# hailanyi/CPD

Measured on AMD Instinct MI355X. Metric: frames/sec voxelize->sparse3D->BEV->NMS, 160k-pt Waymo cloud, higher is better.
Workload: dtype f32 (split-fp16 x2 on the fp16 MFMA pipe: 3 products, fp32 accumulate)

## Files before the change

cpd_amd/_lib.py:

```python
import ctypes
import os

import torch

_HERE = os.path.dirname(os.path.abspath(__file__))
LIB_PATH = os.environ.get("CPD_HIP_LIB", os.path.join(_HERE, "csrc", "libcpd_hip.so"))

CPD_ERRORS = {-1: "CPD_ERR_ARG", -2: "CPD_ERR_WORKSPACE", -3: "CPD_ERR_LAUNCH", -4: "CPD_ERR_UNSUPPORTED"}


class CpdHipError(RuntimeError):
    pass


_lib = None

_VP, _I, _F, _SZ = ctypes.c_void_p, ctypes.c_int, ctypes.c_float, ctypes.c_size_t
_D = ctypes.c_double
_I3 = ctypes.POINTER(ctypes.c_int32)
_FP = ctypes.POINTER(ctypes.c_float)

SIGNATURES = {
    "cpd_launch_log_enable": (None, [_I]),
    "cpd_launch_log_note": (None, [ctypes.c_char_p]),
# ... 4 lines not shown
    "cpd_voxelize_workspace_bytes": (_SZ, [_I, _I, _I, _FP, _FP]),
    "cpd_voxelize_batch_workspace_bytes": (_SZ, [_I, _I, _I, _I, _FP, _FP]),
    "cpd_voxelize_batch": (_I, [_VP, _I3, _I, _I, _FP, _FP, _I, _I, _VP, _VP, _VP, _VP, _VP, _VP, _SZ, _VP]),
    "cpd_voxelize_batch_index": (_I, [_VP, _I3, _I, _I, _FP, _FP, _I, _I, _VP, _VP, _VP, _VP, _VP, _VP, _SZ, _VP, _SZ, _I, _VP]),
    "cpd_voxelize_batch_canonical": (_I, [_VP, _I3, _I, _I, _FP, _FP, _I, _I, _VP, _VP, _VP, _VP, _VP, _VP, _SZ, _VP, _SZ, _I, _VP]),
    "cpd_voxelize_batch_frames": (_I, [_VP, _I3, _I, _I, _FP, _FP, _I, _I, _VP, _VP, _VP, _VP, _VP, _VP, _SZ, _VP, _SZ, _I, _I, _VP]),
    "cpd_voxelize": (_I, [_VP, _I, _I, _FP, _FP, _I, _I, _I, _I, _VP, _VP, _VP, _VP, _VP, _VP, _SZ, _VP]),
    "cpd_index_bytes": (_SZ, [_I, _I3, _I]),
    "cpd_index_build": (_I, [_VP, _I, _I, _I3, _VP, _SZ, _VP]),
    "cpd_order_rows_by_taps_workspace_bytes": (_SZ, [_I]),
    "cpd_order_rows_by_taps": (_I, [_VP, _I, _I, _I3, _I3, _VP, _I, _VP, _VP, _VP, _VP, _SZ, _VP]),
    "cpd_index_set_order": (_I, [_VP, _VP, _VP]),
    "cpd_order_rows_bricks_workspace_bytes": (_SZ, [_I]),
    "cpd_order_rows_bricks": (_I, [_VP, _I, _I, _I3, _VP, _I, _I, _I, _VP, _VP, _VP, _VP, _SZ, _VP]),
    "cpd_rulebook_chunk_ordered": (_I, [_VP, _VP, _I, _I, _I3, _I3, _I3, _I3, _VP, _I, _VP, _VP, _VP]),
    "cpd_rulebook_plan_bytes": (_SZ, [_I, _I, _I]),
    "cpd_rulebook_plan": (_I, [_VP, _I, _I, _I, _VP, _VP, _VP, _VP]),
    "cpd_gather_conv_planned_supported": (_I, [_I, _I, _I, _I, _I, _I, _I]),
    "cpd_gather_conv_planned": (_I, [_VP, _I, _I, _I, _VP, _VP, _VP, _VP, _VP, _I, _I, _I, _I, _VP, _VP, _VP, _I, _I, _VP, _I, _I, _VP, _VP]),
    "cpd_rulebook_subm": (_I, [_VP, _I, _I, _I3, _I3, _VP, _VP, _VP, _VP]),
    "cpd_conv_out_shape": (_I, [_I3, _I3, _I3, _I3, _I3]),
    "cpd_conv_outset": (_I, [_VP, _I, _I, _I3, _I3, _I3, _I3, _VP, _SZ, _VP, _VP]),
    "cpd_index_emit": (_I, [_VP, _I, _I3, _VP, _I, _VP]),
    "cpd_rulebook_conv": (_I, [_VP, _I, _I, _I3, _I3, _I3, _I3, _VP, _VP, _VP, _VP]),
    "cpd_packed_weight_floats": (_SZ, [_I, _I, _I]),
    "cpd_pack_weight": (_I, [_VP, _I, _I, _I, _VP, _VP]),
    "cpd_gather_conv": (_I, [_VP, _I, _I, _I, _VP, _VP, _VP, _I, _I, _I, _VP, _VP, _VP, _I, _I, _VP, _I, _VP, _I, _I, _VP]),
    "cpd_gather_conv_scaled": (_I, [_VP, _I, _I, _I, _VP, _VP, _VP, _I, _I, _I, _VP, _VP, _VP, _I, _I, _VP, _I, _VP, _I, _I, _VP, _VP]),
    "cpd_gather_conv_tile": (_I, [_I, _I, _I, _I, _I] + [ctypes.POINTER(_I)] * 4),
    "cpd_gather_conv_label": (ctypes.c_char_p, [_I, _I, _I, _I, _I, _I, _I]),
# ... 217 lines not shown
```

cpd_amd/csrc/site_index.hip:

```cpp
#include "common.h"

#include "site_index_layout.h"

namespace {

__global__ void __launch_bounds__(256) index_mark_kernel(const int32_t *__restrict__ idx, int n, Grid g, uint64_t *bitmap) {
    int i = blockIdx.x * blockDim.x + threadIdx.x;
    if (i >= n) return;
    int4 q = reinterpret_cast<const int4 *>(idx)[i];
    if ((unsigned)q.x >= (unsigned)g.b || (unsigned)q.y >= (unsigned)g.d || (unsigned)q.z >= (unsigned)g.h ||
        (unsigned)q.w >= (unsigned)g.w)
        return;
    long long k = g.key(q.x, q.y, q.z, q.w);
    atomicOr((unsigned long long *)&bitmap[k >> 6], 1ull << (k & 63));
}

__global__ void __launch_bounds__(256) index_perm_kernel(const int32_t *__restrict__ idx, int n, Grid g,
                                                         const uint64_t *__restrict__ bitmap,
                                                         const uint32_t *__restrict__ base, int32_t *perm) {
    int i = blockIdx.x * blockDim.x + threadIdx.x;
    if (i >= n) return;
    int4 q = reinterpret_cast<const int4 *>(idx)[i];
    if ((unsigned)q.x >= (unsigned)g.b || (unsigned)q.y >= (unsigned)g.d || (unsigned)q.z >= (unsigned)g.h ||
        (unsigned)q.w >= (unsigned)g.w)
// ... 6 lines not shown
    const uint64_t *bitmap;
    __device__ uint32_t operator()(long long w) const { return (uint32_t)__popcll(bitmap[w]); }
};
struct StoreBaseFn {
    uint32_t *base;
    __device__ void operator()(long long w, uint32_t, uint32_t prefix) const { base[w] = prefix; }
};
struct EmitFn {
    const uint64_t *bitmap;
    const uint32_t *base;
    int32_t *out;
    int n_cap;
    Grid g;
    __device__ void operator()(long long wi, uint32_t, uint32_t) const {
        uint64_t w = bitmap[wi];
        uint32_t r = base[wi];
        while (w) {
            int bpos = __ffsll((unsigned long long)w) - 1;
            w &= w - 1;
            long long k = wi * 64 + bpos;
            if ((int)r < n_cap) {
                int x = (int)(k % g.w);
                long long t = k / g.w;
                int y = (int)(t % g.h);
                t /= g.h;
                int z = (int)(t % g.d);
                int bi = (int)(t / g.d);
                reinterpret_cast<int4 *>(out)[r] = make_int4(bi, z, y, x);
            }
            ++r;
        }
    }
};

#pragma clang diagnostic push
#pragma clang diagnostic ignored "-Wpass-failed"
template <bool K3>
__global__ void __launch_bounds__(256)
rulebook_kernel(const int32_t *__restrict__ out_idx, int n_out, Grid gin, int kd_, int kh_, int kw_, int sd, int sh, int sw,
                int pd, int ph, int pw, const uint64_t *__restrict__ bitmap, const uint32_t *__restrict__ base,
                const int32_t *__restrict__ perm_in, const int32_t *__restrict__ flags, int32_t *__restrict__ nbr,
                uint32_t *__restrict__ tapmask, uint32_t *__restrict__ row_pattern) {
    int j = blockIdx.x * blockDim.x + threadIdx.x;
    const int kd = K3 ? 3 : kd_, kh = K3 ? 3 : kh_, kw = K3 ? 3 : kw_;
// ... 11 lines not shown
    for (int tz = 0; tz < kd; ++tz) {
        int z = q.y * sd - pd + tz;
#pragma unroll
        for (int ty = 0; ty < kh; ++ty) {
            int y = q.z * sh - ph + ty;
            const bool row_ok = (unsigned)z < (unsigned)gin.d && (unsigned)y < (unsigned)gin.h && (unsigned)q.x < (unsigned)gin.b &&
                                xlo <= xhi;
            long long rowkey = 0;
            uint64_t wa = 0, wb = 0;
            uint32_t ba = 0, bb = 0;
            long long wia = 0;
            if (row_ok) {
                rowkey = gin.key(q.x, z, y, 0);
                wia = (rowkey + xlo) >> 6;
                const long long wib = (rowkey + xhi) >> 6;
                wa = bitmap[wia]; ba = base[wia];
                wb = wa; bb = ba;
                if (wib != wia) { wb = bitmap[wib]; bb = base[wib]; }
            }
#pragma unroll
            for (int tx = 0; tx < kw; ++tx, ++t) {
                int x = x0 + tx;
                int32_t r = -1;
                if (row_ok && (unsigned)x < (unsigned)gin.w) {
                    const long long k = rowkey + x;
                    const bool first = (k >> 6) == wia;
                    const uint64_t w = first ? wa : wb;
                    const uint64_t bit = 1ull << (k & 63);
                    if (w & bit) {
                        r = (int32_t)((first ? ba : bb) + __popcll(w & (bit - 1ull)));
                        if (perm) r = perm[r];
                    }
                }
                if (live && nbr) nbr[(size_t)t * n_out + j] = r;
                if (r >= 0 && t < 32) pattern |= 1u << t;
                const unsigned long long hit = __ballot(live && r >= 0);
                if (lane < 4 && t < 32 && ((hit >> (16 * lane)) & 0xffffull)) my_mask |= 1u << t;
            }
        }
    }
    if (tapmask && lane < 4) {
        const int sub = ((blockIdx.x * blockDim.x + (threadIdx.x & ~63)) >> 4) + lane;
        if (sub < (n_out + 15) / 16) tapmask[sub] = my_mask;
    }
    if (row_pattern && live) row_pattern[j] = pattern;
}

#pragma clang diagnostic pop

#define CPD_RBC_CHUNK 4096
__global__ void __launch_bounds__(1024)
rulebook_chunk_kernel(const int32_t *__restrict__ out_canon, const int32_t *__restrict__ out_o2n, int n_out, Grid gin, int sd, int sh, int sw,
                      int pd, int ph, int pw, const uint64_t *__restrict__ bitmap, const uint32_t *__restrict__ base,
                      const int32_t *__restrict__ perm_in, const int32_t *__restrict__ flags, int32_t *__restrict__ nbr,
                      uint32_t *__restrict__ tapmask) {
    __shared__ int32_t stage[3][CPD_RBC_CHUNK];
    constexpr int RPT = CPD_RBC_CHUNK / 1024;
    const int tid = threadIdx.x;
    const int c0 = blockIdx.x * CPD_RBC_CHUNK;
    const int32_t *perm = index_order(flags, perm_in);
    int4 q[RPT];
    int dst[RPT];
#pragma unroll
    for (int k = 0; k < RPT; ++k) {
        const int j = c0 + k * 1024 + tid;
        dst[k] = -1;
        q[k] = make_int4(0, 0, 0, 0);
        if (j < n_out) {
            q[k] = reinterpret_cast<const int4 *>(out_canon)[j];
            dst[k] = (out_o2n ? out_o2n[j] : j) - c0;
        }
    }
    uint32_t pattern[RPT];
#pragma unroll
    for (int k = 0; k < RPT; ++k) pattern[k] = 0;
    for (int tzy = 0; tzy < 9; ++tzy) {
        const int tz = tzy / 3, ty = tzy - 3 * tz;
#pragma unroll
        for (int k = 0; k < RPT; ++k) {
            if (dst[k] < 0) continue;
            const int z = q[k].y * sd - pd + tz, y = q[k].z * sh - ph + ty;
            const int x0 = q[k].w * sw - pw;
            int32_t r3[3] = {-1, -1, -1};
            if ((unsigned)z < (unsigned)gin.d && (unsigned)y < (unsigned)gin.h && (unsigned)q[k].x < (unsigned)gin.b) {
                const long long rowkey = gin.key(q[k].x, z, y, 0);
                const int xlo = x0 < 0 ? 0 : x0, xhi = x0 + 2 < gin.w ? x0 + 2 : gin.w - 1;
                if (xlo <= xhi) {
                    const long long wia = (rowkey + xlo) >> 6, wib = (rowkey + xhi) >> 6;
                    const uint64_t wa = bitmap[wia];
                    const uint32_t ba = base[wia];
                    uint64_t wb = wa;
                    uint32_t bb = ba;
                    if (wib != wia) { wb = bitmap[wib]; bb = base[wib]; }
#pragma unroll
                    for (int tx = 0; tx < 3; ++tx) {
                        const int x = x0 + tx;
                        if ((unsigned)x >= (unsigned)gin.w) continue;
                        const long long kk = rowkey + x;
                        const bool first = (kk >> 6) == wia;
                        const uint64_t w = first ? wa : wb;
                        const uint64_t bit = 1ull << (kk & 63);
                        if (w & bit) {
                            int32_t r = (int32_t)((first ? ba : bb) + __popcll(w & (bit - 1ull)));
                            if (perm) r = perm[r];
                            r3[tx] = r;
                        }
                    }
                }
            }
#pragma unroll
            for (int tx = 0; tx < 3; ++tx) stage[tx][dst[k]] = r3[tx];
        }
        __syncthreads();
#pragma unroll
        for (int k = 0; k < RPT; ++k) {
            const int i = k * 1024 + tid, row = c0 + i;
            if (row < n_out) {
#pragma unroll
                for (int tx = 0; tx < 3; ++tx) {
                    const int32_t v = stage[tx][i];
                    nbr[(size_t)(3 * tzy + tx) * n_out + row] = v;
                    if (v >= 0) pattern[k] |= 1u << (3 * tzy + tx);
                }
            }
        }
        __syncthreads();
    }
    if (tapmask) {
#pragma unroll
        for (int k = 0; k < RPT; ++k) {
            uint32_t m = pattern[k];
#pragma unroll
            for (int o = 8; o > 0; o >>= 1) m |= (uint32_t)__shfl_xor((int)m, o, 16);
            const int row = c0 + k * 1024 + tid;
            if ((tid & 15) == 0 && row < n_out) tapmask[row >> 4] = m;
        }
    }
}

__device__ __forceinline__ void outset_flush(uint64_t *bitmap, long long word, uint64_t mask, bool valid) {
    const int lane = threadIdx.x & 63;
    long long key = valid ? word : -1 - lane;
#pragma unroll
    for (int d = 1; d < 64; d <<= 1) {
        const long long k2 = __shfl_up(key, d, 64);
        const uint64_t m2 = __shfl_up(mask, d, 64);
        if (lane >= d && k2 == key) mask |= m2;
    }
    const long long kn = __shfl_down(key, 1, 64);
    const bool tail = lane == 63 || kn != key;
    if (valid && tail && (bitmap[word] & mask) != mask) atomicOr((unsigned long long *)&bitmap[word], (unsigned long long)mask);
// ... 204 lines not shown
                sm.key[pos] = key[e];
                sm.val[pos] = val[e];
            }
            __syncthreads();
#pragma unroll
            for (int e = 0; e < E; ++e) {
                const int i = (wave * E + e) * 64 + lane;
                key[e] = sm.key[i];
                val[e] = sm.val[i];
            }
            __syncthreads();
        }
    }
};

template <int T, int E>
__global__ void __launch_bounds__(T) order_rows_kernel(const uint32_t *__restrict__ pattern, const int32_t *__restrict__ coords, int n,
                                                       int32_t *__restrict__ new_to_old, int32_t *__restrict__ old_to_new,
                                                       int32_t *__restrict__ coords_out, const int32_t *__restrict__ pre_n2o = nullptr) {
    using sort_t = BlockSort27<T, E>;
    __shared__ typename sort_t::Storage storage;
    const int c0 = blockIdx.x * (T * E), tid = threadIdx.x, lane = tid & 63, wave = tid >> 6;
    uint32_t key[E], val[E];
#pragma unroll
    for (int e = 0; e < E; ++e) {
        const int i = (wave * E + e) * 64 + lane, row = c0 + i;
        key[e] = row < n ? (pattern[row] & 0x7ffffffu) : 0x7ffffffu;
        val[e] = (unsigned)i;
    }
    sort_t::sort(key, val, storage);
#pragma unroll
    for (int e = 0; e < E; ++e) {
        const int row = c0 + (wave * E + e) * 64 + lane;
        if (row < n) {
            const int old = c0 + (int)val[e];
            const int canon = pre_n2o ? pre_n2o[old] : old;
            new_to_old[row] = canon;
            old_to_new[canon] = row;
            if (coords_out) reinterpret_cast<int4 *>(coords_out)[row] = reinterpret_cast<const int4 *>(coords)[old];
        }
    }
}
// ... 29 lines not shown

extern "C" size_t cpd_order_rows_by_taps_workspace_bytes(int n) { return (size_t)(n > 0 ? n : 1) * 4; }

extern "C" int cpd_order_rows_by_taps(const int32_t *indices, int n, int batch, const int32_t shape_zyx[3], const int32_t ksize[3],
                                      const void *index, int chunk_rows, int32_t *new_to_old, int32_t *old_to_new,
                                      int32_t *indices_out, void *workspace, size_t workspace_bytes, cpd_stream_t stream) {
    if (!valid_shape(batch, shape_zyx) || n < 0 || !ksize || !index || (n > 0 && (!indices || !new_to_old || !old_to_new || !workspace)))
        return CPD_ERR_ARG;
    for (int d = 0; d < 3; ++d)
        if (ksize[d] <= 0 || !(ksize[d] & 1)) return CPD_ERR_ARG;
    if (ksize[0] * ksize[1] * ksize[2] > 32 || ksize[2] > 32) return CPD_ERR_UNSUPPORTED;
    if (chunk_rows != 1024 && chunk_rows != 4096 && chunk_rows != 8192 && chunk_rows != 16384) return CPD_ERR_UNSUPPORTED;
    if (workspace_bytes < cpd_order_rows_by_taps_workspace_bytes(n)) return CPD_ERR_WORKSPACE;
    if (n == 0) return CPD_OK;
    hipStream_t s = cpd_s(stream);
    uint32_t *pattern = static_cast<uint32_t *>(workspace);
    IndexView v = index_carve(const_cast<void *>(index), batch, shape_zyx, 1);
    Grid g{batch, shape_zyx[0], shape_zyx[1], shape_zyx[2]};
    if (ksize[0] == 3 && ksize[1] == 3 && ksize[2] == 3)
        rulebook_kernel<true><<<cpd_div_up(n, 256), 256, 0, s>>>(indices, n, g, 3, 3, 3, 1, 1, 1, 1, 1, 1, v.bitmap, v.base, v.perm, v.flags,
                                                                 nullptr, nullptr, pattern);
    else
        rulebook_kernel<false><<<cpd_div_up(n, 256), 256, 0, s>>>(indices, n, g, ksize[0], ksize[1], ksize[2], 1, 1, 1, ksize[0] / 2,
                                                                  ksize[1] / 2, ksize[2] / 2, v.bitmap, v.base, v.perm, v.flags, nullptr,
                                                                  nullptr, pattern);
    const int blocks = cpd_div_up(n, chunk_rows);
    if (chunk_rows == 1024) order_rows_kernel<256, 4><<<blocks, 256, 0, s>>>(pattern, indices, n, new_to_old, old_to_new, indices_out);
    else if (chunk_rows == 4096) order_rows_kernel<1024, 4><<<blocks, 1024, 0, s>>>(pattern, indices, n, new_to_old, old_to_new, indices_out);
    else if (chunk_rows == 8192) order_rows_kernel<1024, 8><<<blocks, 1024, 0, s>>>(pattern, indices, n, new_to_old, old_to_new, indices_out);
    else order_rows_kernel<1024, 16><<<blocks, 1024, 0, s>>>(pattern, indices, n, new_to_old, old_to_new, indices_out);
    return cpd_check_launch();
}

struct BrickLayout { size_t pattern, pos_to_row, coords, total; };
static BrickLayout brick_layout(int n) {
    const size_t n1 = (size_t)(n > 0 ? n : 1);
    Carve c;
    BrickLayout l;
    l.pattern = c.take(n1 * 4);
    l.pos_to_row = c.take(n1 * 4);
    l.coords = c.take(n1 * 16);
// ... 11 lines not shown
        (n > 0 && (!indices || !new_to_old || !old_to_new || !indices_out || !workspace)))
        return CPD_ERR_ARG;
    const BrickLayout l = brick_layout(n);
    if (workspace_bytes < l.total) return CPD_ERR_WORKSPACE;
    if (n == 0) return CPD_OK;
    hipStream_t s = cpd_s(stream);
    uint32_t *pattern = ws_at<uint32_t>(workspace, l.pattern);
    int32_t *pos_to_row = ws_at<int32_t>(workspace, l.pos_to_row);
    int32_t *coords_b = ws_at<int32_t>(workspace, l.coords);
    IndexView v = index_carve(const_cast<void *>(index), batch, shape_zyx, 1);
    Grid g{batch, shape_zyx[0], shape_zyx[1], shape_zyx[2]};
    brick_position_kernel<<<cpd_div_up(n, 256), 256, 0, s>>>(indices, n, g, brick_y, brick_x, v.bitmap, v.base, v.bsum, v.words, pos_to_row,
                                                             coords_b);
    rulebook_kernel<true><<<cpd_div_up(n, 256), 256, 0, s>>>(coords_b, n, g, 3, 3, 3, 1, 1, 1, 1, 1, 1, v.bitmap, v.base, v.perm, v.flags,
                                                             nullptr, nullptr, pattern);
    if (tile_rows == 128) order_rows_kernel<64, 2><<<cpd_div_up(n, 128), 64, 0, s>>>(pattern, coords_b, n, new_to_old, old_to_new, indices_out, pos_to_row);
    else order_rows_kernel<64, 4><<<cpd_div_up(n, 256), 64, 0, s>>>(pattern, coords_b, n, new_to_old, old_to_new, indices_out, pos_to_row);
    return cpd_check_launch();
}

extern "C" int cpd_index_set_order(void *index, const int32_t *rank_to_row, cpd_stream_t stream) {
    if (!index) return CPD_ERR_ARG;
    index_set_order_kernel<<<1, 1, 0, cpd_s(stream)>>>(static_cast<int32_t *>(index), rank_to_row);
    return cpd_check_launch();
}

extern "C" int cpd_conv_out_shape(const int32_t in_shape[3], const int32_t ksize[3], const int32_t stride[3],
                                  const int32_t pad[3], int32_t out_shape[3]) {
    if (!in_shape || !ksize || !stride || !pad || !out_shape) return CPD_ERR_ARG;
    for (int d = 0; d < 3; ++d) {
        if (ksize[d] <= 0 || stride[d] <= 0 || pad[d] < 0) return CPD_ERR_ARG;
        out_shape[d] = (in_shape[d] + 2 * pad[d] - ksize[d]) / stride[d] + 1;
// ... 30 lines not shown
    return rulebook_launch(indices, n, batch, shape_zyx, ksize, one, pad, index, nbr, tapmask, cpd_s(stream));
}

extern "C" int cpd_rulebook_conv(const int32_t *out_indices, int n_out, int batch, const int32_t in_shape[3],
                                 const int32_t ksize[3], const int32_t stride[3], const int32_t pad[3],
                                 const void *in_index, int32_t *nbr, uint32_t *tapmask, cpd_stream_t stream) {
    int32_t os[3];
    if (!valid_shape(batch, in_shape) || n_out < 0 || !in_index || (n_out > 0 && (!out_indices || !nbr)))
        return CPD_ERR_ARG;
    int rc = cpd_conv_out_shape(in_shape, ksize, stride, pad, os);
    if (rc) return rc;
    return rulebook_launch(out_indices, n_out, batch, in_shape, ksize, stride, pad, in_index, nbr, tapmask, cpd_s(stream));
}


extern "C" int cpd_rulebook_chunk_ordered(const int32_t *out_canonical, const int32_t *out_old_to_new, int n_out, int batch,
                                          const int32_t in_shape[3], const int32_t ksize[3], const int32_t stride[3], const int32_t pad[3],
                                          const void *in_index, int chunk_rows, int32_t *nbr, uint32_t *tapmask, cpd_stream_t stream) {
    if (!valid_shape(batch, in_shape) || n_out < 0 || !in_index || !ksize || !stride || !pad || (n_out > 0 && (!out_canonical || !nbr)))
        return CPD_ERR_ARG;
    if (ksize[0] != 3 || ksize[1] != 3 || ksize[2] != 3 || chunk_rows != CPD_RBC_CHUNK) return CPD_ERR_UNSUPPORTED;
    if (n_out == 0) return CPD_OK;
    IndexView v = index_carve(const_cast<void *>(in_index), batch, in_shape, 1);
    Grid g{batch, in_shape[0], in_shape[1], in_shape[2]};
    rulebook_chunk_kernel<<<cpd_div_up(n_out, CPD_RBC_CHUNK), 1024, 0, cpd_s(stream)>>>(out_canonical, out_old_to_new, n_out, g, stride[0], stride[1],
                                                                                         stride[2], pad[0], pad[1], pad[2], v.bitmap, v.base, v.perm,
                                                                                         v.flags, nbr, tapmask);
    return cpd_check_launch();
}

extern "C" int cpd_conv_outset(const int32_t *in_indices, int n_in, int batch, const int32_t in_shape[3],
                               const int32_t ksize[3], const int32_t stride[3], const int32_t pad[3], void *out_index,
                               size_t out_index_bytes, int32_t *n_out, cpd_stream_t stream) {
    int32_t os[3];
    if (!valid_shape(batch, in_shape) || n_in < 0 || !out_index || !n_out || (n_in > 0 && !in_indices)) return CPD_ERR_ARG;
    int rc = cpd_conv_out_shape(in_shape, ksize, stride, pad, os);
    if (rc) return rc;
    if (!valid_shape(batch, os)) return CPD_ERR_UNSUPPORTED;
    IndexView v = index_carve(out_index, batch, os, 0);
    if (out_index_bytes < v.bytes) return CPD_ERR_WORKSPACE;
    hipStream_t s = cpd_s(stream);
    Grid g{batch, os[0], os[1], os[2]};
// ... 88 lines not shown
```

cpd_amd/engine.py:

```python
import contextlib
import math
import os
from dataclasses import dataclass, field
from typing import Dict, List, NamedTuple, Optional

import torch

from . import _lib, layer_table, ops, train_ops
from .layer_table import _DOWN, STRIDED_STAGES, final_shape
from .range_guard import GUARDED_BITS, OPTIMISTIC_BITS, BlockPool, RangeGuard


@dataclass
class ModelConfig:
    point_cloud_range: List[float] = field(default_factory=lambda: [-75.2, -75.2, -2.0, 75.2, 75.2, 4.0])
    voxel_size: List[float] = field(default_factory=lambda: [0.1, 0.1, 0.15])
    max_points_per_voxel: int = 5
    max_voxels: int = 1000000
    num_point_features: int = 5
    num_filters: List[int] = field(default_factory=lambda: [16, 32, 64, 128])
    out_features: int = 128
    bev_layer_nums: List[int] = field(default_factory=lambda: [5, 5])
    bev_layer_strides: List[int] = field(default_factory=lambda: [1, 2])
    bev_num_filters: List[int] = field(default_factory=lambda: [128, 256])
# ... 296 lines not shown
            if stage == "conv_out":
                return _StageTables(out_idx, out_index, out_shape, ops.rulebook_conv(out_idx, index, k, s, pd), None, False, None)
            out_c = out_idx
            c_lvl = L[stage + ".down"].c_out
            use_plan = self.cfg.plan_rulebooks and pairs and c_lvl in self.cfg.plan_channels
            bricks = self.cfg.row_order == "bricks" and out_idx.shape[0] >= self.cfg.row_order_min_rows and (use_plan or not self.cfg.plan_rulebooks)
            canon = None
            if bricks:
                out_idx, _, old_to_new = ops.order_rows_bricks(out_c, out_index, brick=self.cfg.row_order_brick, tile_rows=self.cfg.plan_tile_rows)
                out_index.set_order(old_to_new)
            elif self.cfg.row_order in ("taps", "bricks") and out_idx.shape[0] >= self.cfg.row_order_min_rows:
                out_idx, _, old_to_new = ops.order_rows_by_taps(out_c, out_index, chunk_rows=self.cfg.row_order_chunk)
                out_index.set_order(old_to_new)
                if self.cfg.chunked_rulebooks:
                    canon = (out_c, old_to_new, self.cfg.row_order_chunk)
            nbr_dn = ops.rulebook_conv(out_idx, index, k, s, pd, canonical=canon)
            pairs_out = pairs and out_idx.shape[0] * c_lvl * 4 < 0xfffff000
            nbr = ops.rulebook_subm(out_idx, out_index, canonical=canon)
            if bricks and pairs_out and use_plan:
                ops.rulebook_plan(nbr, self.cfg.plan_tile_rows)
            return _StageTables(out_idx, out_index, out_shape, nbr_dn, nbr, pairs_out, canon)

        chain = self._index_chain = StridedStageChain(tables, batch, self.device, side)
        chain.start(coords, shape)
        if index is None:
            index = ops.SiteIndex.build(coords, batch, shape)
        coords_c0, canon0 = coords, None
        if canonical0 and self.cfg.row_order == "taps" and self.cfg.row_order_level0 and coords.shape[0] >= self.cfg.row_order_min_rows:
            coords, n2o, o2n = ops.order_rows_by_taps(coords_c0, index, chunk_rows=self.cfg.row_order_chunk)
            index.set_order(o2n)
            feats = feats.index_select(0, n2o.long())
            if self.cfg.chunked_rulebooks:
                canon0 = (coords_c0, o2n, self.cfg.row_order_chunk)
# ... 294 lines not shown
```

cpd_amd/ops.py:

```python
import ctypes

import torch

from . import _lib
from ._lib import check, farr, iarr, lib, ptr, stream


def _need_cuda(t, name):
    if not t.is_cuda:
        raise _lib.CpdHipError("%s must be a device (HIP) tensor" % name)


def voxel_grid_size(vsize_xyz, range_xyz):
    g = (ctypes.c_int32 * 3)()
    check(lib().cpd_voxel_grid_size(farr(vsize_xyz), farr(range_xyz), g), "cpd_voxel_grid_size")
    return [g[0], g[1], g[2]]


class Voxelizer:

    def __init__(self, vsize_xyz, range_xyz, num_point_features, max_points_per_voxel, max_voxels, device="cuda"):
        self.vs = [float(v) for v in vsize_xyz]
        self.rg = [float(v) for v in range_xyz]
        self.c = int(num_point_features)
# ... 140 lines not shown
    slots = torch.empty((lib().cpd_rulebook_plan_bytes(n, t, 0) // 2,), dtype=torch.int16, device=dev)
    ulist = torch.empty((lib().cpd_rulebook_plan_bytes(n, t, 1) // 4,), dtype=torch.int32, device=dev)
    count = torch.empty((lib().cpd_rulebook_plan_bytes(n, t, 2) // 4,), dtype=torch.int32, device=dev)
    check(lib().cpd_rulebook_plan(ptr(nbr), kv, n, t, ptr(slots), ptr(ulist), ptr(count), stream()), "cpd_rulebook_plan")
    nbr.plan = (slots, ulist, count, t)
    return nbr


def _new_tapmask(n, kv, device):
    if kv > 32 or n == 0:
        return None
    return torch.empty(((n + 15) // 16,), dtype=torch.int32, device=device)


CHUNKED_MIN_ROWS = 200 * 4096


def _rulebook_chunked(canonical, in_index, ksize, stride, pad, n):
    out_c, o2n, chunk = canonical
    dev = out_c.device
    nbr = torch.empty((27, n), dtype=torch.int32, device=dev)
    tapmask = _new_tapmask(n, 27, dev)
    check(lib().cpd_rulebook_chunk_ordered(ptr(out_c.contiguous()), ptr(o2n), n, in_index.batch, iarr(in_index.shape), iarr(ksize), iarr(stride),
                                           iarr(pad), ptr(in_index.buf), int(chunk), ptr(nbr), ptr(tapmask), stream()), "cpd_rulebook_chunk_ordered")
    nbr.tapmask = tapmask
    return nbr


def rulebook_subm(indices, index, ksize=(3, 3, 3), canonical=None):
    if canonical is not None and tuple(ksize) == (3, 3, 3) and canonical[2] == 4096 and indices.shape[0] >= CHUNKED_MIN_ROWS:
        return _rulebook_chunked(canonical, index, ksize, (1, 1, 1), (1, 1, 1), indices.shape[0])
    indices = indices.contiguous()
    n = indices.shape[0]
    kv = int(ksize[0] * ksize[1] * ksize[2])
    nbr = torch.empty((kv, n), dtype=torch.int32, device=indices.device)
    tapmask = _new_tapmask(n, kv, indices.device)
    check(lib().cpd_rulebook_subm(ptr(indices), n, index.batch, iarr(index.shape), iarr(ksize), ptr(index.buf),
                                  ptr(nbr), ptr(tapmask), stream()), "cpd_rulebook_subm")
    nbr.tapmask = tapmask
    return nbr

# ... 714 lines not shown
```

include/cpd_hip.h:

```cpp
#ifndef CPD_HIP_H
#define CPD_HIP_H

#include <stddef.h>
#include <stdint.h>

#ifdef __cplusplus
extern "C" {
#endif

typedef void *cpd_stream_t;

#define CPD_OK 0
#define CPD_ERR_ARG (-1)
#define CPD_ERR_WORKSPACE (-2)
#define CPD_ERR_LAUNCH (-3)
#define CPD_ERR_UNSUPPORTED (-4)

const char *cpd_version(void);
void cpd_launch_log_enable(int on);
void cpd_launch_log_note(const char *kernel);
size_t cpd_launch_log_dump(char *buf, size_t cap);
int cpd_last_hip_error(void);

int cpd_voxel_grid_size(const float vsize_xyz[3], const float range_xyz[6], int32_t grid_zyx[3]);
// ... 40 lines not shown
int cpd_index_set_order(void *index, const int32_t *rank_to_row, cpd_stream_t stream);
size_t cpd_order_rows_bricks_workspace_bytes(int n);
int cpd_order_rows_bricks(const int32_t *indices, int n, int batch, const int32_t shape_zyx[3], const void *index,
                          int brick_y, int brick_x, int tile_rows, int32_t *new_to_old, int32_t *old_to_new, int32_t *indices_out,
                          void *workspace, size_t workspace_bytes, cpd_stream_t stream);
int cpd_rulebook_subm(const int32_t *indices, int n, int batch, const int32_t shape_zyx[3],
                      const int32_t ksize[3], const void *index, int32_t *nbr, uint32_t *tapmask,
                      cpd_stream_t stream);
size_t cpd_rulebook_plan_bytes(int n_out, int tile_rows, int which);
int cpd_rulebook_plan(const int32_t *nbr, int kv, int n_out, int tile_rows, uint16_t *slots, int32_t *ulist, int32_t *count,
                      cpd_stream_t stream);
int cpd_rulebook_chunk_ordered(const int32_t *out_canonical, const int32_t *out_old_to_new, int n_out, int batch,
                               const int32_t in_shape[3], const int32_t ksize[3], const int32_t stride[3],
                               const int32_t pad[3], const void *in_index, int chunk_rows, int32_t *nbr, uint32_t *tapmask,
                               cpd_stream_t stream);
int cpd_conv_out_shape(const int32_t in_shape[3], const int32_t ksize[3], const int32_t stride[3],
                       const int32_t pad[3], int32_t out_shape[3]);
int cpd_conv_outset(const int32_t *in_indices, int n_in, int batch, const int32_t in_shape[3],
                    const int32_t ksize[3], const int32_t stride[3], const int32_t pad[3],
                    void *out_index, size_t out_index_bytes, int32_t *n_out, cpd_stream_t stream);
int cpd_index_emit(const void *index, int batch, const int32_t shape_zyx[3], int32_t *indices,
                   int n_capacity, cpd_stream_t stream);
int cpd_rulebook_conv(const int32_t *out_indices, int n_out, int batch, const int32_t in_shape[3],
                      const int32_t ksize[3], const int32_t stride[3], const int32_t pad[3],
                      const void *in_index, int32_t *nbr, uint32_t *tapmask, cpd_stream_t stream);

size_t cpd_packed_weight_floats(int kv, int c_in, int c_out);
int cpd_pack_weight(const float *w_kio, int kv, int c_in, int c_out, float *packed,
                    cpd_stream_t stream);
int cpd_gather_conv(const float *in, int in_ld, int n_in, int c_in, const float *packed_w,
// ... 469 lines not shown
```

Before: 1233.

## Fuse downsample and submanifold chunked rulebooks into one paired launch with prefetch

Adds a paired chunked rulebook kernel that builds the strided-conv and submanifold neighbour tables for a stage in one launch. It also software-prefetches the next tap row's bitmap words and writes vectorized rows. Separately, the order-by-taps path computes tap patterns inline from the bitmap instead of running a rulebook pass. Index emit now decodes coordinates incrementally, and unneeded base or ballot work is skipped when outputs are null. The paired path is gated on large row counts and adds register pressure.

```diff
diff --git a/cpd_amd/_lib.py b/cpd_amd/_lib.py
--- a/cpd_amd/_lib.py
+++ b/cpd_amd/_lib.py
@@ -42,6 +42,7 @@
     "cpd_order_rows_bricks_workspace_bytes": (_SZ, [_I]),
     "cpd_order_rows_bricks": (_I, [_VP, _I, _I, _I3, _VP, _I, _I, _I, _VP, _VP, _VP, _VP, _SZ, _VP]),
     "cpd_rulebook_chunk_ordered": (_I, [_VP, _VP, _I, _I, _I3, _I3, _I3, _I3, _VP, _I, _VP, _VP, _VP]),
+    "cpd_rulebook_chunk_pair": (_I, [_VP, _VP, _I, _I, _I3, _I3, _I3, _VP, _I3, _VP, _I, _VP, _VP, _VP, _VP, _VP]),
     "cpd_rulebook_plan_bytes": (_SZ, [_I, _I, _I]),
     "cpd_rulebook_plan": (_I, [_VP, _I, _I, _I, _VP, _VP, _VP, _VP]),
     "cpd_gather_conv_planned_supported": (_I, [_I, _I, _I, _I, _I, _I, _I]),
diff --git a/cpd_amd/csrc/site_index.hip b/cpd_amd/csrc/site_index.hip
--- a/cpd_amd/csrc/site_index.hip
+++ b/cpd_amd/csrc/site_index.hip
@@ -1,6 +1,8 @@
 #include "common.h"
 
 #include "site_index_layout.h"
+
+#include <type_traits>
 
 namespace {
 
@@ -44,20 +46,28 @@
     Grid g;
     __device__ void operator()(long long wi, uint32_t, uint32_t) const {
         uint64_t w = bitmap[wi];
+        if (!w) return;
         uint32_t r = base[wi];
+        const long long k0 = wi * 64;
+        int lx = (int)(k0 % g.w);
+        long long t = k0 / g.w;
+        int y = (int)(t % g.h);
+        t /= g.h;
+        int z = (int)(t % g.d);
+        int bi = (int)(t / g.d);
         while (w) {
-            int bpos = __ffsll((unsigned long long)w) - 1;
+            const int bpos = __ffsll((unsigned long long)w) - 1;
             w &= w - 1;
-            long long k = wi * 64 + bpos;
-            if ((int)r < n_cap) {
-                int x = (int)(k % g.w);
-                long long t = k / g.w;
-                int y = (int)(t % g.h);
-                t /= g.h;
-                int z = (int)(t % g.d);
-                int bi = (int)(t / g.d);
-                reinterpret_cast<int4 *>(out)[r] = make_int4(bi, z, y, x);
-            }
+            int x = lx + bpos;
+            while (x >= g.w) {
+                x -= g.w;
+                lx -= g.w;
+                if (++y == g.h) {
+                    y = 0;
+                    if (++z == g.d) { z = 0; ++bi; }
+                }
+            }
+            if ((int)r < n_cap) reinterpret_cast<int4 *>(out)[r] = make_int4(bi, z, y, x);
             ++r;
         }
     }
@@ -99,9 +109,13 @@
                 rowkey = gin.key(q.x, z, y, 0);
                 wia = (rowkey + xlo) >> 6;
                 const long long wib = (rowkey + xhi) >> 6;
-                wa = bitmap[wia]; ba = base[wia];
+                wa = bitmap[wia];
+                if (nbr) ba = base[wia];
                 wb = wa; bb = ba;
-                if (wib != wia) { wb = bitmap[wib]; bb = base[wib]; }
+                if (wib != wia) {
+                    wb = bitmap[wib];
+                    if (nbr) bb = base[wib];
+                }
             }
 #pragma unroll
             for (int tx = 0; tx < kw; ++tx, ++t) {
@@ -113,14 +127,19 @@
                     const uint64_t w = first ? wa : wb;
                     const uint64_t bit = 1ull << (k & 63);
                     if (w & bit) {
-                        r = (int32_t)((first ? ba : bb) + __popcll(w & (bit - 1ull)));
-                        if (perm) r = perm[r];
+                        r = 0;
+                        if (nbr) {
+                            r = (int32_t)((first ? ba : bb) + __popcll(w & (bit - 1ull)));
+                            if (perm) r = perm[r];
+                        }
                     }
                 }
                 if (live && nbr) nbr[(size_t)t * n_out + j] = r;
                 if (r >= 0 && t < 32) pattern |= 1u << t;
-                const unsigned long long hit = __ballot(live && r >= 0);
-                if (lane < 4 && t < 32 && ((hit >> (16 * lane)) & 0xffffull)) my_mask |= 1u << t;
+                if (tapmask) {
+                    const unsigned long long hit = __ballot(live && r >= 0);
+                    if (lane < 4 && t < 32 && ((hit >> (16 * lane)) & 0xffffull)) my_mask |= 1u << t;
+                }
             }
         }
     }
@@ -134,92 +153,147 @@
 #pragma clang diagnostic pop
 
 #define CPD_RBC_CHUNK 4096
+struct ChunkTable {
+    Grid gin;
+    int sd, sh, sw, pd, ph, pw;
+    const uint64_t *bitmap;
+    const uint32_t *base;
+    const int32_t *perm_in, *flags;
+    int32_t *nbr;
+    uint32_t *tapmask;
+};
+template <int NT>
+struct ChunkTables { ChunkTable t[NT]; };
+struct __attribute__((packed, aligned(4))) Row4 { int32_t v[4]; };
+
+template <int NT>
 __global__ void __launch_bounds__(1024)
-rulebook_chunk_kernel(const int32_t *__restrict__ out_canon, const int32_t *__restrict__ out_o2n, int n_out, Grid gin, int sd, int sh, int sw,
-                      int pd, int ph, int pw, const uint64_t *__restrict__ bitmap, const uint32_t *__restrict__ base,
-                      const int32_t *__restrict__ perm_in, const int32_t *__restrict__ flags, int32_t *__restrict__ nbr,
-                      uint32_t *__restrict__ tapmask) {
+rulebook_chunk_kernel(const int32_t *__restrict__ out_canon, const int32_t *__restrict__ out_o2n, int n_out, ChunkTables<NT> tabs) {
     __shared__ int32_t stage[3][CPD_RBC_CHUNK];
     constexpr int RPT = CPD_RBC_CHUNK / 1024;
+    struct TapWords { uint64_t wa, wb; uint32_t ba, bb; };
     const int tid = threadIdx.x;
-    const int c0 = blockIdx.x * CPD_RBC_CHUNK;
-    const int32_t *perm = index_order(flags, perm_in);
-    int4 q[RPT];
-    int dst[RPT];
+    const int c0 = (int)(blockIdx.x / NT) * CPD_RBC_CHUNK;
+    const ChunkTable &a = tabs.t[blockIdx.x % NT];
+    const Grid gin = a.gin;
+    const uint64_t *__restrict__ bitmap = a.bitmap;
+    const uint32_t *__restrict__ base = a.base;
+    int32_t *__restrict__ nbr = a.nbr;
+    const int32_t *perm = index_order(a.flags, a.perm_in);
+    long long key0[RPT];
+    int x0[RPT], dst[RPT];
+    uint32_t lines[RPT];
 #pragma unroll
     for (int k = 0; k < RPT; ++k) {
         const int j = c0 + k * 1024 + tid;
         dst[k] = -1;
-        q[k] = make_int4(0, 0, 0, 0);
+        key0[k] = 0;
+        x0[k] = 0;
+        lines[k] = 0;
         if (j < n_out) {
-            q[k] = reinterpret_cast<const int4 *>(out_canon)[j];
+            const int4 q = reinterpret_cast<const int4 *>(out_canon)[j];
             dst[k] = (out_o2n ? out_o2n[j] : j) - c0;
-        }
-    }
+            const int z0 = q.y * a.sd - a.pd, y0 = q.z * a.sh - a.ph;
+            x0[k] = q.w * a.sw - a.pw;
+            key0[k] = gin.key(q.x, z0, y0, 0);
+            if ((unsigned)q.x < (unsigned)gin.b && x0[k] + 2 >= 0 && x0[k] < gin.w)
+#pragma unroll
+                for (int t = 0; t < 9; ++t)
+                    if ((unsigned)(z0 + t / 3) < (unsigned)gin.d && (unsigned)(y0 + t % 3) < (unsigned)gin.h) lines[k] |= 1u << t;
+        }
+    }
+    auto fetch = [&](int tzy, TapWords (&w)[RPT]) {
+        const long long off = (long long)((tzy / 3) * gin.h + tzy % 3) * gin.w;
+#pragma unroll
+        for (int k = 0; k < RPT; ++k) {
+            const bool ok = (lines[k] >> tzy) & 1u;
+            const int xlo = x0[k] < 0 ? 0 : x0[k], xhi = x0[k] + 2 < gin.w ? x0[k] + 2 : gin.w - 1;
+            const long long rowkey = key0[k] + off;
+            const long long wia = ok ? (rowkey + xlo) >> 6 : 0, wib = ok ? (rowkey + xhi) >> 6 : 0;
+            w[k].wa = bitmap[wia];
+            w[k].ba = base[wia];
+            w[k].wb = 0ull;
+            w[k].bb = 0u;
+            if (wib != wia) { w[k].wb = bitmap[wib]; w[k].bb = base[wib]; }
+        }
+    };
+    static_assert(RPT == 4, "the read-out below takes four rows per lane");
     uint32_t pattern[RPT];
 #pragma unroll
     for (int k = 0; k < RPT; ++k) pattern[k] = 0;
-    for (int tzy = 0; tzy < 9; ++tzy) {
-        const int tz = tzy / 3, ty = tzy - 3 * tz;
+    TapWords words[RPT];
+    auto drop = [&](auto hp, int tzy) {
+        constexpr bool HP = decltype(hp)::value;
+        const uint32_t off = (uint32_t)(((tzy / 3) * gin.h + tzy % 3) * gin.w);
+        int32_t r[RPT][3];
+#pragma unroll
+        for (int k = 0; k < RPT; ++k) {
+            const bool ok = (lines[k] >> tzy) & 1u;
+            const int xlo = x0[k] < 0 ? 0 : x0[k];
+            const int sh = (int)(((uint32_t)key0[k] + off + (uint32_t)xlo) & 63u);
+#pragma unroll
+            for (int tx = 0; tx < 3; ++tx) {
+                const int x = x0[k] + tx;
+                const int bp = sh + (x - xlo);
+                const bool first = bp < 64;
+                const uint64_t ww = first ? words[k].wa : words[k].wb;
+                const uint64_t bit = 1ull << (bp & 63);
+                const bool hit = ok && (unsigned)x < (unsigned)gin.w && (ww & bit);
+                const int32_t rank = (int32_t)((first ? words[k].ba : words[k].bb) + __popcll(ww & (bit - 1ull)));
+                if (HP) {
+                    const int32_t v = perm[hit ? rank : 0];
+                    r[k][tx] = hit ? v : -1;
+                } else {
+                    r[k][tx] = hit ? rank : -1;
+                }
+            }
+        }
 #pragma unroll
         for (int k = 0; k < RPT; ++k) {
             if (dst[k] < 0) continue;
-            const int z = q[k].y * sd - pd + tz, y = q[k].z * sh - ph + ty;
-            const int x0 = q[k].w * sw - pw;
-            int32_t r3[3] = {-1, -1, -1};
-            if ((unsigned)z < (unsigned)gin.d && (unsigned)y < (unsigned)gin.h && (unsigned)q[k].x < (unsigned)gin.b) {
-                const long long rowkey = gin.key(q[k].x, z, y, 0);
-                const int xlo = x0 < 0 ? 0 : x0, xhi = x0 + 2 < gin.w ? x0 + 2 : gin.w - 1;
-                if (xlo <= xhi) {
-                    const long long wia = (rowkey + xlo) >> 6, wib = (rowkey + xhi) >> 6;
-                    const uint64_t wa = bitmap[wia];
-                    const uint32_t ba = base[wia];
-                    uint64_t wb = wa;
-                    uint32_t bb = ba;
-                    if (wib != wia) { wb = bitmap[wib]; bb = base[wib]; }
-#pragma unroll
-                    for (int tx = 0; tx < 3; ++tx) {
-                        const int x = x0 + tx;
-                        if ((unsigned)x >= (unsigned)gin.w) continue;
-                        const long long kk = rowkey + x;
-                        const bool first = (kk >> 6) == wia;
-                        const uint64_t w = first ? wa : wb;
-                        const uint64_t bit = 1ull << (kk & 63);
-                        if (w & bit) {
-                            int32_t r = (int32_t)((first ? ba : bb) + __popcll(w & (bit - 1ull)));
-                            if (perm) r = perm[r];
-                            r3[tx] = r;
-                        }
-                    }
-                }
-            }
-#pragma unroll
-            for (int tx = 0; tx < 3; ++tx) stage[tx][dst[k]] = r3[tx];
-        }
+#pragma unroll
+            for (int tx = 0; tx < 3; ++tx) stage[tx][dst[k]] = r[k][tx];
+        }
+    };
+    fetch(0, words);
+#pragma unroll 1
+    for (int tzy = 0; tzy < 9; ++tzy) {
+        if (perm) drop(std::true_type{}, tzy);
+        else drop(std::false_type{}, tzy);
+        if (tzy + 1 < 9) fetch(tzy + 1, words);
         __syncthreads();
-#pragma unroll
-        for (int k = 0; k < RPT; ++k) {
-            const int i = k * 1024 + tid, row = c0 + i;
-            if (row < n_out) {
+        const int i0 = 4 * tid, row0 = c0 + i0;
+        if (row0 + RPT <= n_out) {
+#pragma unroll
+            for (int tx = 0; tx < 3; ++tx) {
+                const int4 v = *reinterpret_cast<const int4 *>(&stage[tx][i0]);
+                *reinterpret_cast<Row4 *>(nbr + (size_t)(3 * tzy + tx) * n_out + row0) = Row4{{v.x, v.y, v.z, v.w}};
+                const uint32_t bit = 1u << (3 * tzy + tx);
+                if (v.x >= 0) pattern[0] |= bit;
+                if (v.y >= 0) pattern[1] |= bit;
+                if (v.z >= 0) pattern[2] |= bit;
+                if (v.w >= 0) pattern[3] |= bit;
+            }
+        } else {
+#pragma unroll
+            for (int k = 0; k < RPT; ++k) {
+                if (row0 + k >= n_out) continue;
 #pragma unroll
                 for (int tx = 0; tx < 3; ++tx) {
-                    const int32_t v = stage[tx][i];
-                    nbr[(size_t)(3 * tzy + tx) * n_out + row] = v;
+                    const int32_t v = stage[tx][i0 + k];
+                    nbr[(size_t)(3 * tzy + tx) * n_out + row0 + k] = v;
                     if (v >= 0) pattern[k] |= 1u << (3 * tzy + tx);
                 }
             }
         }
         __syncthreads();
     }
-    if (tapmask) {
-#pragma unroll
-        for (int k = 0; k < RPT; ++k) {
-            uint32_t m = pattern[k];
-#pragma unroll
-            for (int o = 8; o > 0; o >>= 1) m |= (uint32_t)__shfl_xor((int)m, o, 16);
-            const int row = c0 + k * 1024 + tid;
-            if ((tid & 15) == 0 && row < n_out) tapmask[row >> 4] = m;
-        }
+    if (a.tapmask) {
+        uint32_t m = pattern[0] | pattern[1] | pattern[2] | pattern[3];
+        m |= (uint32_t)__shfl_xor((int)m, 1, 4);
+        m |= (uint32_t)__shfl_xor((int)m, 2, 4);
+        const int row0 = c0 + 4 * tid;
+        if ((tid & 3) == 0 && row0 < n_out) a.tapmask[row0 >> 4] = m;
     }
 }
 
@@ -454,8 +528,37 @@
     }
 };
 
-template <int T, int E>
-__global__ void __launch_bounds__(T) order_rows_kernel(const uint32_t *__restrict__ pattern, const int32_t *__restrict__ coords, int n,
+struct StoredKey {
+    const uint32_t *__restrict__ pattern;
+    __device__ uint32_t operator()(int row, const int32_t *) const { return pattern[row]; }
+};
+struct Taps27Key {
+    const uint64_t *__restrict__ bitmap;
+    Grid g;
+    __device__ uint32_t operator()(int row, const int32_t *__restrict__ coords) const {
+        const int4 q = reinterpret_cast<const int4 *>(coords)[row];
+        const int x0 = q.w - 1;
+        const int xlo = x0 < 0 ? 0 : x0, xhi = x0 + 2 < g.w ? x0 + 2 : g.w - 1;
+        if ((unsigned)q.x >= (unsigned)g.b || xlo > xhi) return 0u;
+        const uint32_t keep = ((1u << (xhi - xlo + 1)) - 1u) << (xlo - x0);
+        uint32_t pattern = 0;
+#pragma unroll
+        for (int tzy = 0; tzy < 9; ++tzy) {
+            const int tz = tzy / 3, ty = tzy - 3 * tz;
+            const int z = q.y - 1 + tz, y = q.z - 1 + ty;
+            if ((unsigned)z >= (unsigned)g.d || (unsigned)y >= (unsigned)g.h) continue;
+            const long long klo = g.key(q.x, z, y, xlo), khi = klo + (xhi - xlo);
+            const int sh = (int)(klo & 63);
+            uint64_t v = bitmap[klo >> 6] >> sh;
+            if ((khi >> 6) != (klo >> 6)) v |= bitmap[khi >> 6] << (64 - sh);
+            pattern |= (((uint32_t)v << (xlo - x0)) & keep) << (3 * tzy);
+        }
+        return pattern;
+    }
+};
+
+template <int T, int E, class KeyFn>
+__global__ void __launch_bounds__(T) order_rows_kernel(KeyFn key_of, const int32_t *__restrict__ coords, int n,
                                                        int32_t *__restrict__ new_to_old, int32_t *__restrict__ old_to_new,
                                                        int32_t *__restrict__ coords_out, const int32_t *__restrict__ pre_n2o = nullptr) {
     using sort_t = BlockSort27<T, E>;
@@ -465,7 +568,7 @@
 #pragma unroll
     for (int e = 0; e < E; ++e) {
         const int i = (wave * E + e) * 64 + lane, row = c0 + i;
-        key[e] = row < n ? (pattern[row] & 0x7ffffffu) : 0x7ffffffu;
+        key[e] = row < n ? (key_of(row, coords) & 0x7ffffffu) : 0x7ffffffu;
         val[e] = (unsigned)i;
     }
     sort_t::sort(key, val, storage);
@@ -525,17 +628,23 @@
     if (workspace_bytes < cpd_order_rows_by_taps_workspace_bytes(n)) return CPD_ERR_WORKSPACE;
     if (n == 0) return CPD_OK;
     hipStream_t s = cpd_s(stream);
-    uint32_t *pattern = static_cast<uint32_t *>(workspace);
     IndexView v = index_carve(const_cast<void *>(index), batch, shape_zyx, 1);
     Grid g{batch, shape_zyx[0], shape_zyx[1], shape_zyx[2]};
-    if (ksize[0] == 3 && ksize[1] == 3 && ksize[2] == 3)
+    const int blocks = cpd_div_up(n, chunk_rows);
+    const bool k3 = ksize[0] == 3 && ksize[1] == 3 && ksize[2] == 3;
+    if (k3 && chunk_rows == 4096) {
+        order_rows_kernel<1024, 4><<<blocks, 1024, 0, s>>>(Taps27Key{v.bitmap, g}, indices, n, new_to_old, old_to_new, indices_out);
+        return cpd_check_launch();
+    }
+    StoredKey pattern{static_cast<uint32_t *>(workspace)};
+    uint32_t *pattern_out = static_cast<uint32_t *>(workspace);
+    if (k3)
         rulebook_kernel<true><<<cpd_div_up(n, 256), 256, 0, s>>>(indices, n, g, 3, 3, 3, 1, 1, 1, 1, 1, 1, v.bitmap, v.base, v.perm, v.flags,
-                                                                 nullptr, nullptr, pattern);
+                                                                 nullptr, nullptr, pattern_out);
     else
         rulebook_kernel<false><<<cpd_div_up(n, 256), 256, 0, s>>>(indices, n, g, ksize[0], ksize[1], ksize[2], 1, 1, 1, ksize[0] / 2,
                                                                   ksize[1] / 2, ksize[2] / 2, v.bitmap, v.base, v.perm, v.flags, nullptr,
-                                                                  nullptr, pattern);
-    const int blocks = cpd_div_up(n, chunk_rows);
+                                                                  nullptr, pattern_out);
     if (chunk_rows == 1024) order_rows_kernel<256, 4><<<blocks, 256, 0, s>>>(pattern, indices, n, new_to_old, old_to_new, indices_out);
     else if (chunk_rows == 4096) order_rows_kernel<1024, 4><<<blocks, 1024, 0, s>>>(pattern, indices, n, new_to_old, old_to_new, indices_out);
     else if (chunk_rows == 8192) order_rows_kernel<1024, 8><<<blocks, 1024, 0, s>>>(pattern, indices, n, new_to_old, old_to_new, indices_out);
@@ -577,8 +686,8 @@
                                                              coords_b);
     rulebook_kernel<true><<<cpd_div_up(n, 256), 256, 0, s>>>(coords_b, n, g, 3, 3, 3, 1, 1, 1, 1, 1, 1, v.bitmap, v.base, v.perm, v.flags,
                                                              nullptr, nullptr, pattern);
-    if (tile_rows == 128) order_rows_kernel<64, 2><<<cpd_div_up(n, 128), 64, 0, s>>>(pattern, coords_b, n, new_to_old, old_to_new, indices_out, pos_to_row);
-    else order_rows_kernel<64, 4><<<cpd_div_up(n, 256), 64, 0, s>>>(pattern, coords_b, n, new_to_old, old_to_new, indices_out, pos_to_row);
+    if (tile_rows == 128) order_rows_kernel<64, 2><<<cpd_div_up(n, 128), 64, 0, s>>>(StoredKey{pattern}, coords_b, n, new_to_old, old_to_new, indices_out, pos_to_row);
+    else order_rows_kernel<64, 4><<<cpd_div_up(n, 256), 64, 0, s>>>(StoredKey{pattern}, coords_b, n, new_to_old, old_to_new, indices_out, pos_to_row);
     return cpd_check_launch();
 }
 
@@ -639,6 +748,13 @@
 }
 
 
+static ChunkTable chunk_table(int batch, const int32_t in_shape[3], const int32_t stride[3], const int32_t pad[3], const void *in_index,
+                              int32_t *nbr, uint32_t *tapmask) {
+    IndexView v = index_carve(const_cast<void *>(in_index), batch, in_shape, 1);
+    return ChunkTable{Grid{batch, in_shape[0], in_shape[1], in_shape[2]}, stride[0], stride[1], stride[2], pad[0], pad[1], pad[2],
+                      v.bitmap, v.base, v.perm, v.flags, nbr, tapmask};
+}
+
 extern "C" int cpd_rulebook_chunk_ordered(const int32_t *out_canonical, const int32_t *out_old_to_new, int n_out, int batch,
                                           const int32_t in_shape[3], const int32_t ksize[3], const int32_t stride[3], const int32_t pad[3],
                                           const void *in_index, int chunk_rows, int32_t *nbr, uint32_t *tapmask, cpd_stream_t stream) {
@@ -646,11 +762,24 @@
         return CPD_ERR_ARG;
     if (ksize[0] != 3 || ksize[1] != 3 || ksize[2] != 3 || chunk_rows != CPD_RBC_CHUNK) return CPD_ERR_UNSUPPORTED;
     if (n_out == 0) return CPD_OK;
-    IndexView v = index_carve(const_cast<void *>(in_index), batch, in_shape, 1);
-    Grid g{batch, in_shape[0], in_shape[1], in_shape[2]};
-    rulebook_chunk_kernel<<<cpd_div_up(n_out, CPD_RBC_CHUNK), 1024, 0, cpd_s(stream)>>>(out_canonical, out_old_to_new, n_out, g, stride[0], stride[1],
-                                                                                         stride[2], pad[0], pad[1], pad[2], v.bitmap, v.base, v.perm,
-                                                                                         v.flags, nbr, tapmask);
+    ChunkTables<1> tabs{{chunk_table(batch, in_shape, stride, pad, in_index, nbr, tapmask)}};
+    rulebook_chunk_kernel<1><<<cpd_div_up(n_out, CPD_RBC_CHUNK), 1024, 0, cpd_s(stream)>>>(out_canonical, out_old_to_new, n_out, tabs);
+    return cpd_check_launch();
+}
+
+extern "C" int cpd_rulebook_chunk_pair(const int32_t *out_canonical, const int32_t *out_old_to_new, int n_out, int batch,
+                                       const int32_t in_shape[3], const int32_t stride[3], const int32_t pad[3], const void *in_index,
+                                       const int32_t out_shape[3], const void *out_index, int chunk_rows, int32_t *nbr_down,
+                                       uint32_t *tapmask_down, int32_t *nbr_subm, uint32_t *tapmask_subm, cpd_stream_t stream) {
+    if (!valid_shape(batch, in_shape) || !valid_shape(batch, out_shape) || n_out < 0 || !in_index || !out_index || !stride || !pad ||
+        (n_out > 0 && (!out_canonical || !nbr_down || !nbr_subm)))
+        return CPD_ERR_ARG;
+    if (chunk_rows != CPD_RBC_CHUNK) return CPD_ERR_UNSUPPORTED;
+    if (n_out == 0) return CPD_OK;
+    const int32_t one[3] = {1, 1, 1};
+    ChunkTables<2> tabs{{chunk_table(batch, in_shape, stride, pad, in_index, nbr_down, tapmask_down),
+                         chunk_table(batch, out_shape, one, one, out_index, nbr_subm, tapmask_subm)}};
+    rulebook_chunk_kernel<2><<<2 * cpd_div_up(n_out, CPD_RBC_CHUNK), 1024, 0, cpd_s(stream)>>>(out_canonical, out_old_to_new, n_out, tabs);
     return cpd_check_launch();
 }
 
diff --git a/cpd_amd/engine.py b/cpd_amd/engine.py
--- a/cpd_amd/engine.py
+++ b/cpd_amd/engine.py
@@ -334,9 +334,10 @@
                 out_index.set_order(old_to_new)
                 if self.cfg.chunked_rulebooks:
                     canon = (out_c, old_to_new, self.cfg.row_order_chunk)
-            nbr_dn = ops.rulebook_conv(out_idx, index, k, s, pd, canonical=canon)
+            both = ops.rulebook_stage_chunked(canon, index, s, pd, out_index) if canon is not None and tuple(k) == (3, 3, 3) else None
+            nbr_dn = both[0] if both else ops.rulebook_conv(out_idx, index, k, s, pd, canonical=canon)
             pairs_out = pairs and out_idx.shape[0] * c_lvl * 4 < 0xfffff000
-            nbr = ops.rulebook_subm(out_idx, out_index, canonical=canon)
+            nbr = both[1] if both else ops.rulebook_subm(out_idx, out_index, canonical=canon)
             if bricks and pairs_out and use_plan:
                 ops.rulebook_plan(nbr, self.cfg.plan_tile_rows)
             return _StageTables(out_idx, out_index, out_shape, nbr_dn, nbr, pairs_out, canon)
diff --git a/cpd_amd/ops.py b/cpd_amd/ops.py
--- a/cpd_amd/ops.py
+++ b/cpd_amd/ops.py
@@ -178,6 +178,7 @@
 
 
 CHUNKED_MIN_ROWS = 200 * 4096
+PAIR_MAX_ROWS = 1024 * 4096
 
 
 def _rulebook_chunked(canonical, in_index, ksize, stride, pad, n):
@@ -189,6 +190,21 @@
                                            iarr(pad), ptr(in_index.buf), int(chunk), ptr(nbr), ptr(tapmask), stream()), "cpd_rulebook_chunk_ordered")
     nbr.tapmask = tapmask
     return nbr
+
+
+def rulebook_stage_chunked(canonical, in_index, stride, pad, out_index):
+    out_c, o2n, chunk = canonical
+    n = out_c.shape[0]
+    if chunk != 4096 or n < CHUNKED_MIN_ROWS or n > PAIR_MAX_ROWS:
+        return None
+    dev = out_c.device
+    nbr_dn = torch.empty((27, n), dtype=torch.int32, device=dev)
+    nbr = torch.empty((27, n), dtype=torch.int32, device=dev)
+    nbr_dn.tapmask, nbr.tapmask = _new_tapmask(n, 27, dev), _new_tapmask(n, 27, dev)
+    check(lib().cpd_rulebook_chunk_pair(ptr(out_c.contiguous()), ptr(o2n), n, in_index.batch, iarr(in_index.shape), iarr(stride), iarr(pad),
+                                        ptr(in_index.buf), iarr(out_index.shape), ptr(out_index.buf), int(chunk), ptr(nbr_dn),
+                                        ptr(nbr_dn.tapmask), ptr(nbr), ptr(nbr.tapmask), stream()), "cpd_rulebook_chunk_pair")
+    return nbr_dn, nbr
 
 
 def rulebook_subm(indices, index, ksize=(3, 3, 3), canonical=None):
diff --git a/include/cpd_hip.h b/include/cpd_hip.h
--- a/include/cpd_hip.h
+++ b/include/cpd_hip.h
@@ -78,6 +78,10 @@
                                const int32_t in_shape[3], const int32_t ksize[3], const int32_t stride[3],
                                const int32_t pad[3], const void *in_index, int chunk_rows, int32_t *nbr, uint32_t *tapmask,
                                cpd_stream_t stream);
+int cpd_rulebook_chunk_pair(const int32_t *out_canonical, const int32_t *out_old_to_new, int n_out, int batch,
+                            const int32_t in_shape[3], const int32_t stride[3], const int32_t pad[3], const void *in_index,
+                            const int32_t out_shape[3], const void *out_index, int chunk_rows, int32_t *nbr_down,
+                            uint32_t *tapmask_down, int32_t *nbr_subm, uint32_t *tapmask_subm, cpd_stream_t stream);
 int cpd_conv_out_shape(const int32_t in_shape[3], const int32_t ksize[3], const int32_t stride[3],
                        const int32_t pad[3], int32_t out_shape[3]);
 int cpd_conv_outset(const int32_t *in_indices, int n_in, int batch, const int32_t in_shape[3],
```

Measured after the change: 1249 (median of 5 runs). 1.3% higher.
